# anthonyhu/tumblr-emotions

Hardware: AMD Instinct MI355X
Metric: training samples/sec (224x224 img + 32-tok text, batch 256) (higher is better)
Workload: dtype f32; 1 GPU; joint train step (fwd+bwd+all-reduce+Adam): Inception-v1 224x224x3 + 300-d embedding + LSTM-512, T=32, V=10000, 15 classes, batch 256 per GPU, reference freeze (<=Mixed_5b conv weights frozen, all BN betas trainable), dropout 0.8, BN train mode; global_batch=256, per_gpu_batch=256, parallelism=dp1, launch=eager

## Files before the change

### include/ds_kernels.h

```cpp
#ifndef DS_KERNELS_H
#define DS_KERNELS_H

#include <stddef.h>
#include <stdint.h>

#ifdef __cplusplus
extern "C" {
#endif

#define DS_OK 0
#define DS_ERR_ARG (-1)
#define DS_ERR_LAUNCH (-2)
#define DS_ERR_WORKSPACE (-3)

#define DS_DTYPE_F32 0
#define DS_DTYPE_BF16 1

#define DS_EPI_BIAS 1
#define DS_EPI_RELU 2
#define DS_EPI_ACCUM 4
#define DS_EPI_STATS 8
#define DS_EPI_MASK 16
#define DS_EPI_BNSUMS 32
#define DS_EPI_BN_RELU 64
// ... 20 lines not shown
    int32_t splits;
    int64_t z_split_stride;
    int32_t tile_nt;
    int32_t grid_x;
    int32_t dtype;
    int32_t x_dtype;
    int32_t partials;
    const float *norm_rstd;
    const float *norm_shift;
    const float *mask_rstd;
    const float *mask_shift;
    const struct ds_bn_bwd_on_load *bnb;
    int32_t mask_dtype;
    int32_t z_dtype;
    uint8_t *pool_argmax;
    const struct ds_bn_finalize_in_launch *fin;
} ds_conv_desc;

typedef struct ds_bn_finalize_in_launch {
    const float *beta;
    float *mean, *rstd, *shift;
    float *moving_mean, *moving_var;
    uint32_t *ticket;
    int64_t count;
    float eps, decay;
} ds_bn_finalize_in_launch;

typedef struct ds_bn_bwd_on_load {
    const float *mean, *rstd, *shift;
    const float *coef;
// ... 7 lines not shown
int ds_debug_conv_set_tile(int mt, int nt);
int ds_debug_conv_set_path(int path);
int ds_debug_conv_set_wide(int mode);
int ds_debug_conv_wino_allow_ablation(int on);
int ds_debug_conv_wino4_set_nb(int nb);
int ds_debug_conv_bf16_set_max_nb(int nb);
int ds_debug_conv_wgrad_force(int ai, int bj, int slabs);
int ds_debug_conv_wgrad_plan(const ds_conv_desc *d, const float *x, const float *dz, int32_t lddz, const float *dw,
                             const void *ws, int out[6]);
#endif
int ds_conv_igemm_partials(const ds_conv_desc *d);
int ds_conv_igemm_bnsums_supported(const ds_conv_desc *d);
int ds_conv_igemm_norm_supported(const ds_conv_desc *d);
int ds_conv_igemm_bnb_supported(const ds_conv_desc *d);
int ds_conv_igemm_pool3_supported(const ds_conv_desc *d);
int ds_conv_igemm_finalize_tickets(const ds_conv_desc *d);
int ds_conv_igemm(const ds_conv_desc *d, const float *x, const float *w, float *z, const float *bias,
                  const float *mask, float *stats, const float *pivot, void *stream);

size_t ds_weights_bf16_bytes(int32_t Cin, int32_t Cout, int32_t taps, int32_t dgrad);
int ds_weights_to_bf16(const float *w, void *wb, int32_t Cin, int32_t Cout, int32_t taps, int32_t dgrad, void *stream);
int ds_conv_bf16_supported(const ds_conv_desc *d);
int ds_conv_bf16_partials(const ds_conv_desc *d);
int ds_conv_bf16(const ds_conv_desc *d, const void *x, const void *wb, float *z, const void *mask, float *stats,
                 const float *pivot, void *stream);

size_t ds_weights_f32x3_bytes(int32_t Cin, int32_t Cout, int32_t taps, int32_t dgrad);
int ds_weights_to_f32x3(const float *w, void *wb, int32_t Cin, int32_t Cout, int32_t taps, int32_t dgrad, void *stream);
int ds_conv_f32x3_supported(const ds_conv_desc *d);
int ds_conv_f32x3_partials(const ds_conv_desc *d);
// ... 105 lines not shown
    const float *x_amax;
    const float *wscale;
    const ds_bn_finalize_in_launch *fin;
    void *ws;
    size_t ws_bytes;
    const float *scale;
    const float *shift;
} ds_conv_io;
int ds_conv_plan(ds_conv_layer_plan *plan, int32_t role, int32_t arith, uint32_t options, int32_t N, int32_t H, int32_t W,
                 int32_t w_cin, int32_t w_cout, int32_t k, int32_t stride, int32_t ldx, int32_t ldz, int32_t flags);
int ds_conv_plan_set_flags(ds_conv_layer_plan *plan, int32_t flags);
int ds_conv_plan_enable_bnsums(ds_conv_layer_plan *plan, int32_t ldy);
int ds_conv_plan_norm_supported(const ds_conv_layer_plan *plan);
int ds_conv_plan_bnb_supported(const ds_conv_layer_plan *plan);
int ds_conv_plan_enable_pool3(ds_conv_layer_plan *plan, uint8_t *argmax);
int ds_conv_plan_enable_bn_relu(ds_conv_layer_plan *plan);
int ds_conv_plan_finalize_tickets(const ds_conv_layer_plan *plan);
int ds_conv_prepare_weights(const ds_conv_layer_plan *plan, const float *w_hwio, void *w_prepared, float *wscale,
                            void *stream);
int ds_conv_run(const ds_conv_layer_plan *plan, const void *x, const void *w, float *z, const ds_conv_io *io, void *stream);

size_t ds_conv_wgrad_workspace(const ds_conv_desc *d);
int ds_conv_wgrad(const ds_conv_desc *d, const float *x, const float *dz, int32_t lddz, float *dw,
                  void *ws, size_t ws_bytes, void *stream);

int ds_bn_finalize(const float *stats, int32_t P, int64_t count, int32_t C, const float *beta, const float *pivot,
                   float eps, float decay, float *mean, float *rstd, float *shift, float *moving_mean,
                   float *moving_var, void *stream);

int ds_bn_finalize_centered(const float *stats, int32_t P, int64_t count, int32_t C, const float *beta, const float *pivot,
// ... 349 lines not shown
```

### tumblr_emotions_amd/_lib.py

```python
import ctypes as C
import os

_HERE = os.path.dirname(os.path.abspath(__file__))
LIB_PATH = os.environ.get("DS_LIB") or os.path.join(_HERE, "libds_kernels.so")

def tuning_env(name, default=None):
    return os.environ.get(name, default) if os.environ.get("DS_LIB") else default


DS_EPI_BIAS, DS_EPI_RELU, DS_EPI_ACCUM, DS_EPI_STATS, DS_EPI_MASK, DS_EPI_BNSUMS = 1, 2, 4, 8, 16, 32
DS_EPI_BN_RELU = 64
DS_DTYPE_F32, DS_DTYPE_BF16 = 0, 1
DS_FP8_E4M3, DS_FP8_E5M2 = 0, 1
DS_CONV_FWD, DS_CONV_DGRAD = 0, 1
DS_LSTM_SKIP_MASKED = 256
DS_ARITH_F32, DS_ARITH_BF16, DS_ARITH_FP8, DS_ARITH_F32X3 = 0, 1, 2, 3
DS_FAM_IGEMM, DS_FAM_WINO2, DS_FAM_WINO4, DS_FAM_STEM, DS_FAM_BF16D, DS_FAM_FP8D, DS_FAM_F32X3, DS_FAM_WINO4H, DS_FAM_STEM_POOL = range(9)
DS_FAM_STEM_DGRAD = 9
DS_PLAN_NO_WINO, DS_PLAN_NO_WINO4, DS_PLAN_NO_STEM_DIRECT, DS_PLAN_NO_BF16_DIRECT, DS_PLAN_ACT16, DS_PLAN_PACKED_RGB = 1, 2, 4, 8, 16, 32
DS_PLAN_FP8_EVERYWHERE, DS_PLAN_FP8_WIDE_RULE, DS_PLAN_NO_WINO4H, DS_PLAN_STEM_POOL = 64, 128, 256, 512
DS_PLAN_NO_SPLITK = 1024
DS_PREPROCESS_FLIP, DS_PREPROCESS_SATURATION_FIRST = 1, 2
DS_JPEG_UNSUPPORTED, DS_JPEG_MORE = 1, 2
DS_JPEG_444, DS_JPEG_422, DS_JPEG_420, DS_JPEG_GREY = 0, 1, 2, 3
DS_JPEG_E_CODE, DS_JPEG_E_RUN, DS_JPEG_E_RANGE, DS_JPEG_E_COLUMN, DS_JPEG_E_SEGMENT, DS_JPEG_E_TABLE = 1, 2, 4, 8, 16, 32


class ConvDesc(C.Structure):
    _fields_ = [
        ("N", C.c_int32), ("H", C.c_int32), ("W", C.c_int32), ("Cin", C.c_int32), ("ldx", C.c_int32),
        ("KH", C.c_int32), ("KW", C.c_int32), ("stride", C.c_int32), ("pad_t", C.c_int32), ("pad_l", C.c_int32),
        ("OH", C.c_int32), ("OW", C.c_int32), ("Cout", C.c_int32), ("ldz", C.c_int32),
        ("w_tap_stride", C.c_int64), ("w_n_stride", C.c_int32), ("w_k_stride", C.c_int32),
        ("flip", C.c_int32), ("fold_cin", C.c_int32), ("flags", C.c_int32), ("ldmask", C.c_int32),
        ("splits", C.c_int32), ("z_split_stride", C.c_int64),
        ("tile_nt", C.c_int32), ("grid_x", C.c_int32), ("dtype", C.c_int32), ("x_dtype", C.c_int32),
        ("partials", C.c_int32),
        ("norm_rstd", C.c_void_p), ("norm_shift", C.c_void_p), ("mask_rstd", C.c_void_p), ("mask_shift", C.c_void_p),
        ("bnb", C.c_void_p), ("mask_dtype", C.c_int32), ("z_dtype", C.c_int32), ("pool_argmax", C.c_void_p), ("fin", C.c_void_p),
    ]


class BnBwdOnLoad(C.Structure):
    _fields_ = [("mean", C.c_void_p), ("rstd", C.c_void_p), ("shift", C.c_void_p), ("coef", C.c_void_p),
                ("nseg", C.c_int32), ("c_end", C.c_int32 * 3), ("ld", C.c_int32 * 3), ("dy", C.c_void_p * 3)]


class BnFinalizeInLaunch(C.Structure):
    _fields_ = [("beta", C.c_void_p), ("mean", C.c_void_p), ("rstd", C.c_void_p), ("shift", C.c_void_p),
                ("moving_mean", C.c_void_p), ("moving_var", C.c_void_p), ("ticket", C.c_void_p), ("count", C.c_int64),
                ("eps", C.c_float), ("decay", C.c_float)]


class LayerPlanStruct(C.Structure):
# ... 90 lines not shown
_i32, _i64, _f32, _u64 = C.c_int32, C.c_int64, C.c_float, C.c_uint64
_CD = C.POINTER(ConvDesc)
_SG = C.POINTER(Segments)
_SS = C.POINTER(SumSegments)
_LP = C.POINTER(LayerPlanStruct)
_IO = C.POINTER(ConvIO)

SIGNATURES = {
    "ds_version": (C.c_int, []),
    "ds_last_error": (C.c_char_p, []),
    "ds_conv_igemm_partials": (C.c_int, [_CD]),
    "ds_conv_igemm_bnsums_supported": (C.c_int, [_CD]),
    "ds_conv_igemm_norm_supported": (C.c_int, [_CD]),
    "ds_conv_igemm_bnb_supported": (C.c_int, [_CD]),
    "ds_conv_igemm_pool3_supported": (C.c_int, [_CD]),
    "ds_conv_igemm_finalize_tickets": (C.c_int, [_CD]),
    "ds_conv_igemm": (C.c_int, [_CD, _P, _P, _P, _P, _P, _P, _P, _P]),
    "ds_weights_bf16_bytes": (C.c_size_t, [_i32, _i32, _i32, _i32]),
    "ds_weights_to_bf16": (C.c_int, [_P, _P, _i32, _i32, _i32, _i32, _P]),
    "ds_conv_bf16_supported": (C.c_int, [_CD]),
    "ds_conv_bf16_partials": (C.c_int, [_CD]),
    "ds_conv_bf16": (C.c_int, [_CD, _P, _P, _P, _P, _P, _P, _P]),
    "ds_weights_f32x3_bytes": (C.c_size_t, [_i32, _i32, _i32, _i32]),
    "ds_weights_to_f32x3": (C.c_int, [_P, _P, _i32, _i32, _i32, _i32, _P]),
    "ds_conv_f32x3_supported": (C.c_int, [_CD]),
    "ds_conv_f32x3_partials": (C.c_int, [_CD]),
    "ds_conv_f32x3": (C.c_int, [_CD, _P, _P, _P, _P, _P, _P, _P]),
    "ds_absmax": (C.c_int, [_P, _i64, _i32, _P, _P]),
    "ds_weights_fp8_bytes": (C.c_size_t, [_i32, _i32, _i32, _i32]),
    "ds_weights_to_fp8": (C.c_int, [_P, _P, _P, _i32, _i32, _i32, _i32, _P]),
# ... 19 lines not shown
    "ds_conv_wino4_partials": (C.c_int, [_i32, _i32, _i32]),
    "ds_conv_wino4_splitk_choose": (C.c_int, [_i32, _i32, _i32, _i32, _i32]),
    "ds_conv_wino4_splitk_partials": (C.c_int, [_i32, _i32, _i32]),
    "ds_conv_wino4_splitk_workspace": (C.c_size_t, [_i32, _i32, _i32, _i32, _i32]),
    "ds_conv_wino4_splitk": (C.c_int, [_P, _P, _P, _P, _P, _P, _i32, _i32, _i32, _i32, _i32, _i32, _i32, _i32, _i32, _i32, _P, C.c_size_t, _P]),
    "ds_conv_wino4": (C.c_int, [_P, _P, _P, _P, _P, _P, _i32, _i32, _i32, _i32, _i32, _i32, _i32, _i32, _P]),
    "ds_conv_wino4_bf16x2": (C.c_int, [_P, _P, _P, _P, _P, _P, _i32, _i32, _i32, _i32, _i32, _i32, _i32, _i32, _i32, _P]),
    "ds_conv_wino4_bf16x2_x16": (C.c_int, [_P, _P, _P, _P, _P, _P, _i32, _i32, _i32, _i32, _i32, _i32, _i32, _i32, _i32, _P]),
    "ds_wino4_transform_weights_bf16x2": (C.c_int, [_P, _P, _i32, _i32, _i32, _P]),
    "ds_conv_plan": (C.c_int, [_LP, _i32, _i32, C.c_uint32] + [_i32] * 10),
    "ds_conv_plan_set_flags": (C.c_int, [_LP, _i32]),
    "ds_conv_plan_enable_bnsums": (C.c_int, [_LP, _i32]),
    "ds_conv_plan_norm_supported": (C.c_int, [_LP]),
    "ds_conv_plan_bnb_supported": (C.c_int, [_LP]),
    "ds_conv_plan_enable_pool3": (C.c_int, [_LP, C.c_void_p]),
    "ds_conv_plan_enable_bn_relu": (C.c_int, [_LP]),
    "ds_conv_plan_finalize_tickets": (C.c_int, [_LP]),
    "ds_conv_prepare_weights": (C.c_int, [_LP, _P, _P, _P, _P]),
    "ds_conv_run": (C.c_int, [_LP, _P, _P, _P, _IO, _P]),
    "ds_conv_wgrad_workspace": (C.c_size_t, [_CD]),
    "ds_conv_wgrad": (C.c_int, [_CD, _P, _P, _i32, _P, _P, C.c_size_t, _P]),
    "ds_bn_finalize": (C.c_int, [_P, _i32, _i64, _i32, _P, _P, _f32, _f32, _P, _P, _P, _P, _P, _P]),
    "ds_bn_finalize_centered": (C.c_int, [_P, _i32, _i64, _i32, _P, _P, _f32, _f32, _P, _P, _P, _P, _P, _P, _P, _P]),
    "ds_bn_apply_relu": (C.c_int, [_P, _i64, _i32, _P, _P, _SG, _P]),
    "ds_bn_apply_relu_z16": (C.c_int, [_P, _i64, _i32, _P, _P, _SG, _P]),
    "ds_bn_bwd_apply_z16": (C.c_int, [_P, _i32, _SG, _i64, _i32, _P, _P, _P, _P, _P, _i32, _P, _P]),
    "ds_bn_infer_prepare": (C.c_int, [_P, _P, _P, _f32, _i32, _P, _P, _P]),
    "ds_bn_infer_prepare_multi": (C.c_int, [_P, _i32, _f32, _P]),
    "ds_bn_bwd_partials": (C.c_int, [_i64, _i32]),
    "ds_bn_bwd_reduce": (C.c_int, [_P, _i32, _i32, _SG, _i64, _i32, _P, _P, _P, _P, _P]),
# ... 152 lines not shown
```

### tumblr_emotions_amd/csrc/conv_igemm.hip

```cpp
#include <stdlib.h>
#include <mutex>
#include <type_traits>
#include <unordered_map>
#include "conv_epilogue.h"

using ds::f32x16;
typedef float f32x4 __attribute__((ext_vector_type(4)));
typedef float f32x2 __attribute__((ext_vector_type(2)));
typedef unsigned int u32x4 __attribute__((ext_vector_type(4)));
typedef __attribute__((address_space(3))) void *lds_ptr;

namespace {

constexpr int BK = 16;
constexpr int LDK = 20;
using ds::kOOB;
using ds::make_srd;

struct ConvParams {
    ds_conv_desc d;
    const float *x;
    const float *w;
    float *z;
    const float *bias;
    const float *mask;
// ... 1813 lines not shown
    if (d->splits <= 1) p.d.z_split_stride = 0;
    p.x = (const float *)x; p.w = (const float *)w; p.z = z; p.mask = (const float *)mask; p.stats = stats;
    p.pivot = (d->flags & DS_EPI_STATS) ? pivot : nullptr;
    p.M = (int)conv_M(d);
    p.taps = d->KH * d->KW;
    const int64_t x_elems = ((int64_t)d->N * d->H * d->W - 1) * d->ldx + (d->fold_cin > 0 ? d->fold_cin : d->Cin);
    const int64_t w_elems = (int64_t)(p.taps - 1) * d->w_tap_stride + (int64_t)(d->Cout - 1) * d->w_n_stride +
                            (int64_t)(d->Cin - 1) * d->w_k_stride + 1;
    const int64_t w_bytes = prepared_w_bytes < 0 ? w_elems * 4 : prepared_w_bytes;
    DS_REQUIRE(x_elems * 4 < (1ll << 31) && w_bytes < (1ll << 31), "%s: operand larger than 2 GiB%s", who, hint);
    p.x_bytes = (unsigned)(x_elems * 4);
    p.w_bytes = (unsigned)w_bytes;
    return DS_OK;
}

int igemm_launch(const ds_conv_desc *d, const float *x, const float *w, float *z, const float *bias, const float *mask,
                 float *stats, const float *pivot, const float *scale, const float *shift, void *stream) {
    DS_REQUIRE(d && x && w && z, "ds_conv_igemm: null argument");
    DS_REQUIRE(d->Cin > 0 && d->Cout > 0 && d->N > 0 && d->OH > 0 && d->OW > 0, "ds_conv_igemm: bad dims");
    DS_REQUIRE(d->w_n_stride == 1 || d->w_k_stride == 1, "ds_conv_igemm: one weight stride must be 1");
    DS_REQUIRE(!(d->flags & DS_EPI_BIAS) || bias, "ds_conv_igemm: DS_EPI_BIAS without bias");
    DS_REQUIRE(!(d->flags & DS_EPI_MASK) || mask, "ds_conv_igemm: DS_EPI_MASK without mask");
    DS_REQUIRE(!(d->flags & DS_EPI_STATS) || stats, "ds_conv_igemm: DS_EPI_STATS without stats buffer");
    DS_REQUIRE(!(d->flags & DS_EPI_BNSUMS) || (stats && mask && !(d->flags & (DS_EPI_STATS | DS_EPI_MASK)) && d->ldmask >= d->Cout),
               "ds_conv_igemm: DS_EPI_BNSUMS needs the partials buffer (stats), y (mask, ldmask) and excludes STATS / MASK");
    DS_REQUIRE(conv_M(d) < (1ll << 31), "ds_conv_igemm: M too large");
    DS_REQUIRE(d->dtype == DS_DTYPE_F32 || d->dtype == DS_DTYPE_BF16, "ds_conv_igemm: dtype must be DS_DTYPE_F32 or DS_DTYPE_BF16");
    const Launch L = choose(d, aligned16(x, w));
    const Variant &v = L.v;
    const TileCfg &c = L.c;
    DS_REQUIRE(!(d->flags & DS_EPI_STATS) || v.vec == dims_vec(d),
               "ds_conv_igemm: DS_EPI_STATS needs 16-byte aligned operand pointers");

    ConvParams p;
// ... 89 lines not shown
extern "C" int ds_conv_igemm_bnsums_supported(const ds_conv_desc *d) {
    if (!d) return 0;
    ds_conv_desc t = *d;
    t.flags = (t.flags & DS_EPI_ACCUM) | DS_EPI_BNSUMS;
    return choose(&t, true).c.wide > 0 ? 1 : 0;
}

extern "C" int ds_conv_igemm_norm_supported(const ds_conv_desc *d) {
    if (!d || d->Cin > 1024) return 0;
    return choose(d, true).c.wide > 0 ? 1 : 0;
}

extern "C" int ds_conv_igemm_pool3_supported(const ds_conv_desc *d) {
    if (!d) return 0;
    return choose(d, true, kBeforePool).c.wide > 0 ? 1 : 0;
}

extern "C" int ds_conv_igemm_finalize_tickets(const ds_conv_desc *d) {
    if (!d || !(d->flags & DS_EPI_STATS)) return 0;
    ds_conv_desc t = *d;
    t.partials = 0;
    t.fin = nullptr;
    const Launch L = choose(&t, true);
    return L.c.wide && L.row_tiles <= 256 ? L.gy : 0;
}

namespace ds {
int conv_igemm_bn_relu_supported(const ds_conv_desc *d) {
    if (!d || (d->flags & ~DS_EPI_BN_RELU)) return 0;
    ds_conv_desc t = *d;
// ... 184 lines not shown
```

### tumblr_emotions_amd/csrc/conv_plan.cpp

```cpp
#include <stdlib.h>
#include <string.h>

#include "ds_kernels.h"

namespace ds {
void set_error(const char *fmt, ...);
int conv_igemm_bn_relu_supported(const ds_conv_desc *d);
int conv_igemm_bn_relu(const ds_conv_desc *d, const float *x, const float *w, float *z, const float *scale, const float *shift,
                       void *stream);
int conv_wino_bn_relu(const float *x, const float *u, float *z, const float *scale, const float *shift, int32_t N, int32_t H,
                      int32_t W, int32_t Cin, int32_t ldx, int32_t Cout, int32_t ldz, void *stream);
int conv_wino4_bn_relu(const float *x, const float *u, float *z, const float *scale, const float *shift, int32_t N, int32_t H,
                       int32_t W, int32_t Cin, int32_t ldx, int32_t Cout, int32_t ldz, int32_t splits, void *ws, size_t ws_bytes,
                       void *stream);
}

#define PLAN_REQUIRE(cond, ...)         \
    do {                                \
        if (!(cond)) {                  \
            ds::set_error(__VA_ARGS__); \
            return DS_ERR_ARG;          \
        }                               \
    } while (0)

namespace {

// ... 205 lines not shown
extern "C" int ds_conv_plan_bnb_supported(const ds_conv_layer_plan *p) {
    if (p == nullptr || p->role != DS_CONV_DGRAD || p->family != DS_FAM_IGEMM || p->k != 1) return 0;
    const ds_conv_desc t = igemm_desc(p);
    return ds_conv_igemm_bnb_supported(&t);
}

extern "C" int ds_conv_plan_enable_pool3(ds_conv_layer_plan *p, uint8_t *argmax) {
    if (p == nullptr || argmax == nullptr || p->role != DS_CONV_FWD || p->family != DS_FAM_IGEMM || p->k != 1) return 0;
    const ds_conv_desc t = igemm_desc(p);
    if (!ds_conv_igemm_pool3_supported(&t)) return 0;
    p->d.pool_argmax = argmax;
    recount_partials(p);
    return 1;
}

extern "C" int ds_conv_plan_enable_bn_relu(ds_conv_layer_plan *p) {
    if (p == nullptr || p->role != DS_CONV_FWD || p->d.dtype != DS_DTYPE_F32 || p->d.flags != 0) return 0;
    if (p->family == DS_FAM_IGEMM) {
        const ds_conv_desc t = igemm_desc(p);
        if (!ds::conv_igemm_bn_relu_supported(&t)) return 0;
    } else if (p->family == DS_FAM_WINO4) {
        if (p->d.ldz % 4 != 0 || p->d.ldz < p->d.Cout) return 0;
    } else if (p->family != DS_FAM_WINO2) {
        return 0;
    }
    p->d.flags = DS_EPI_BN_RELU;
    p->d.partials = 0;
    p->partials = 0;
    return 1;
}
// ... 98 lines not shown
```

### tumblr_emotions_amd/engine_image.py

```python
import contextlib
import ctypes as C
import os
from collections import namedtuple

import torch

from . import _lib, ops
from .ops import WgradPlan, gemm_plan, make_segments, same_pad, DS_EPI_BIAS, DS_EPI_STATS

BN_EPS = 0.001
BN_DECAY = 0.9997
WEIGHT_DECAY = 0.00004

TOPOLOGY = [
    ("conv", "Conv2d_1a_7x7", 7, 2, 64),
    ("maxpool", "MaxPool_2a_3x3", 3, 2),
    ("conv", "Conv2d_2b_1x1", 1, 1, 64),
    ("conv", "Conv2d_2c_3x3", 3, 1, 192),
    ("maxpool", "MaxPool_3a_3x3", 3, 2),
    ("mixed", "Mixed_3b", 64, (96, 128), (16, 32), 32),
    ("mixed", "Mixed_3c", 128, (128, 192), (32, 96), 64),
    ("maxpool", "MaxPool_4a_3x3", 3, 2),
    ("mixed", "Mixed_4b", 192, (96, 208), (16, 48), 64),
    ("mixed", "Mixed_4c", 160, (112, 224), (24, 64), 64),
# ... 745 lines not shown
        b0, b1a, b1b, b2a, b2b, b3 = self.b
        cin, Ct = self.prev.C, self.C
        self.B = B
        M = B * self.H * self.W
        for l in self.layers:
            l.alloc(B)
        out16 = eng.act16 and self.name not in ("Mixed_5b", "Mixed_5c")
        r16 = eng.act16 and self.name != "Mixed_5c"
        a16 = lambda f: torch.bfloat16 if f else torch.float32
        self.out = torch.empty(B, self.H, self.W, Ct, device=dev, dtype=a16(out16))
        self.dout = torch.empty(B, self.H, self.W, Ct, device=dev)
        self.r1 = torch.empty(M, b1a, device=dev, dtype=a16(r16))
        self.r2 = torch.empty(M, b2a, device=dev, dtype=a16(r16))
        self.dr1 = torch.empty(M, b1a, device=dev)
        self.dr2 = torch.empty(M, b2a, device=dev)
        self.dpooled = torch.empty(M, cin, device=dev)
        self.argmax = torch.empty(M, cin, dtype=torch.uint8, device=dev)
        self.fuse_b3 = bool(eng.fuse_branch3 and not self.c3.trainable and eng.dtype == "f32" and not eng.act16
                            and self.c3.fwd.enable_pool3(self.argmax))
        if self.fuse_b3:
            eng.need_stats(self.c3.fwd.partials * 2 * b3)
        self.pooled = None if self.fuse_b3 else torch.empty(M, cin, device=dev, dtype=self.prev.out.dtype)
        o, do = self.out.data_ptr(), self.dout.data_ptr()
        nf = b0 + b1a + b2a
        es, dt_o, dt_r = self.out.element_size(), ops.act_dtype(self.out), ops.act_dtype(self.r1)
        self.out_amax, self.r1_amax, self.r2_amax = eng.new_amax(), eng.new_amax(), eng.new_amax()
        am_o, am_1, am_2 = ops._p(self.out_amax), ops._p(self.r1_amax), ops._p(self.r2_amax)
        self.seg_f = make_segments([(0, b0, o, Ct, dt_o, am_o), (b0, b0 + b1a, self.r1.data_ptr(), b1a, dt_r, am_1),
                                    (b0 + b1a, nf, self.r2.data_ptr(), b2a, dt_r, am_2)])
        self.seg_1, self.seg_2, self.seg_3 = (make_segments([(0, layer.cout, o + es * off, Ct, dt_o, am_o)])
                                              for layer, off in self.concat_layers()[1:])
# ... 30 lines not shown
        self.fused.make_dgrad(cin, allow_z16=True)
        self.c1.make_dgrad(b1a, allow_z16=True)
        self.c2.make_dgrad(b2a, allow_z16=True)
        self.c3.make_dgrad(cin, allow_z16=True)
        self.dpooled16 = bool(eng.dpooled16 and eng.act16 and self.c3.dgrad.family == ops.DS_FAM_BF16D)
        if self.dpooled16:
            self.dpooled = torch.empty(M, cin, device=dev, dtype=torch.bfloat16)
            self.c3.dgrad.d.z_dtype = ops.DS_DTYPE_BF16
        for part, (layer, r) in enumerate(((self.c1, self.r1), (self.c2, self.r2)), start=1):
            src = layer.emit_dx_sums(r)
            if src is not None:
                self.fused.sums_from(part, src)
        p = self.prev
        fams = (ops.DS_FAM_IGEMM, ops.DS_FAM_BF16D, ops.DS_FAM_FP8D) if _lib.tuning_env("DS_POOL_FIRST_16") == "1" else (ops.DS_FAM_IGEMM,)
        self.pool_first = bool(eng.pool_first and self.fused.dgrad.family in fams)
        if isinstance(p, MixedStage) and self.pool_first:
            src = self.fused.emit_dx_sums(p.out)
            if src is not None and p.zcat:
                self.fused.dgrad.d.mask_rstd = p.rs_cat[0].data_ptr()
                self.fused.dgrad.d.mask_shift = p.rs_cat[1].data_ptr()
            if src is not None:
                for layer, off in p.concat_layers():
                    layer.sums_from(0, src._replace(off=off))
        self.pool_sums = None
        self.split_dout = False
        if isinstance(p, MixedStage) and not self.pool_first and eng.bwd_sums and eng.pool_sums and cin <= 1024 \
                and not p.zcat:
            P = ops.maxpool3_bwd_sums_partials(B, p.W, cin)
            self.pool_sums = torch.empty(2 * cin * P, device=dev)
            src, delta = None, 0
# ... 122 lines not shown
        if self.eng.fuse_fin_apply:
            ops.bn_bwd_finalize_apply(sg, M, Cb, None, None, self.coef_cat, z, dy, self.mean_cat[b0:], self.rs_cat[0, b0:],
                                      self.rs_cat[1, b0:], z, self.fa_ticket, ldz=Ct, betas=[l.beta for l in layers],
                                      dbetas=[l.gbeta for l in layers])
        else:
            ops.bn_bwd_finalize_multi(sg, M, Cb, [l.beta for l in layers], [l.gbeta for l in layers], self.coef_cat)
            if from_pool:
                nx = self.next
                ops.bn_pool_bwd_apply_cols(z, Ct, z, Ct, nx.dout, nx.argmax, Ct, b0, self.B, self.H, self.W, Cb, self.mean_cat[b0:],
                                           self.rs_cat[0, b0:], self.rs_cat[1, b0:], self.coef_cat[0], self.coef_cat[1], nx.k)
            else:
                ops.bn_bwd_apply(z, dy, M, Cb, self.mean_cat[b0:], self.rs_cat[0, b0:], self.rs_cat[1, b0:], self.coef_cat, z, ldz=Ct)
        for l in layers:
            l._dz_amax_live = False

    def forward(self):
        p = self.prev
        b0, b1a, b1b, b2a, b2b, b3 = self.b
        x = ops._p(p.out)
        dx_, dr_ = ops.act_dtype(p.out), ops.act_dtype(self.r1)
        ax_, a1_, a2_ = p.out_amax, self.r1_amax, self.r2_amax
        defer = self._batch_forward()

        def branch3():
            self._pool_fwd()
            self.c3.forward(x if self.fuse_b3 else ops._p(self.pooled), p.C, self.seg_3, dx_, ax_, defer)

        self._fork_join(lambda: self.fused.forward(x, p.C, self.seg_f, dx_, ax_),
                        lambda: self.c1.forward(ops._p(self.r1), b1a, self.seg_1, dr_, a1_, defer),
                        lambda: self.c2.forward(ops._p(self.r2), b2a, self.seg_2, dr_, a2_, defer), branch3)
# ... 31 lines not shown
                        l.fz_job = (self._fz_close.data_ptr() + 4 * off * P, P)
                        off += l.cout
                ops.bn_infer_bwd_apply_sums(z, dy, M, Ct - b0, self.rs_cat[0, b0:], self.rs_cat[1, b0:], z, self._fz_close, ldz=Ct)
            else:
                ops.bn_infer_bwd_apply(z, dy, M, Ct - b0, self.rs_cat[0, b0:], self.rs_cat[1, b0:], z, ldz=Ct)

        def closing(layer, x_ptr, ldx, dx_ptr, ndx):
            if infer:
                layer.backward_pointwise(x_ptr, ldx, dx_ptr, ndx, apply=not self.zcat)
            elif batched:
                layer._run_dgrad(dx_ptr)
            else:
                layer.backward(x_ptr, ldx, dx_ptr, ndx)

        def branch3():
            closing(self.c3, None if self.fuse_b3 else ops._p(self.pooled), p.C, ops._p(self.dpooled), need_dx)
            if pool_first:
                ops.maxpool_bwd(self.dpooled, self.argmax, p.dout, False, self.B, p.H, p.W, p.C, 3, 1, "SAME")
            elif need_dx and self.split_dout and infer:
                ops.maxpool_bwd(self.dpooled, self.argmax, p.dout2, False, self.B, p.H, p.W, p.C, 3, 1, "SAME")
            elif need_dx and self.split_dout:
                ops.maxpool3_bwd_sums(self.dpooled, self.argmax, p.dout2, False, p.out, self.B, p.H, p.W, p.C, self.pool_sums)

        self._fork_join(None, lambda: closing(self.c1, ops._p(self.r1), b1a, ops._p(self.dr1), True),
                        lambda: closing(self.c2, ops._p(self.r2), b2a, ops._p(self.dr2), True), branch3)
        if infer:
            self.fused.backward_pointwise(x, p.C, ops._p(p.dout) if need_dx else None, need_dx)
            if need_dx and not pool_first and not self.split_dout:
                ops.maxpool_bwd(self.dpooled, self.argmax, p.dout, True, self.B, p.H, p.W, p.C, 3, 1, "SAME")
            return
        self.fused.backward(x, p.C, ops._p(p.dout) if need_dx else None, need_dx, pool=self.next if from_pool else None)
        if need_dx and self.split_dout:
            ops.bn_bwd_reduce(p.out, self._dgrad_sum_segs, self.B * p.H * p.W, p.C, eng.zeros, eng.ones, eng.zeros, self.dgrad_sums,
                              ldz=p.C)
        if need_dx and not pool_first and not self.split_dout:
            if self.pool_sums is not None:
                ops.maxpool3_bwd_sums(self.dpooled, self.argmax, p.dout, True, p.out, self.B, p.H, p.W, p.C, self.pool_sums)
            else:
                ops.maxpool_bwd(self.dpooled, self.argmax, p.dout, True, self.B, p.H, p.W, p.C, 3, 1, "SAME")


class InceptionV1Engine:

    def __init__(self, store, num_classes, image_size=224, dropout_keep_prob=0.8, trainable_bn_beta=True,
                 device="cuda", train_all=False, dtype="f32"):
        self.store, self.num_classes, self.keep = store, num_classes, dropout_keep_prob
        assert dtype in ("f32", "bf16", "fp8")
        self.dtype = dtype
        self.conv_dtype = ops.DS_DTYPE_F32 if dtype == "f32" else ops.DS_DTYPE_BF16
        self.trainable_bn_beta = trainable_bn_beta
        self.train_all = train_all
        self.device = torch.device(device)
        self.update_moving = True
        self.training = True
# ... 22 lines not shown
        self.winograd = True
        self.mul3 = _lib.tuning_env("DS_MUL3", "0") == "1"
        self.bnb_on_load = int(_lib.tuning_env("DS_BNB", "1"))
        self.zcat = _lib.tuning_env("DS_ZCAT", "1") != "0"
        self.pool_apply = _lib.tuning_env("DS_POOL_APPLY", "1") != "0"
        self.fuse_finalize = _lib.tuning_env("DS_FUSE_FIN", "0") == "1"
        self.fuse_fin_apply = _lib.tuning_env("DS_FIN_APPLY", "0") == "1"
        e = _lib.tuning_env("DS_BATCH_BN")
        self.batch_bn = int(e) if e else None
        self.pool_sums = _lib.tuning_env("DS_POOL_SUMS", "1") != "0"
        self.split_dout = _lib.tuning_env("DS_SPLIT_DOUT", "0") == "1"
        self.z16 = _lib.tuning_env("DS_Z16", "1") != "0"
        self.dpooled16 = _lib.tuning_env("DS_DPOOLED16", "0") == "1"
        self.stem_sums_from_dgrad = _lib.tuning_env("DS_STEM_SUMS", "1") != "0"
        self.dz16 = int(_lib.tuning_env("DS_DZ16", "2"))
        self.fuse_branch3 = _lib.tuning_env("DS_FUSE_B3", "1") != "0"
        self.winograd4 = _lib.tuning_env("DS_WINO4", "1") != "0"
        self.splitk = _lib.tuning_env("DS_SPLITK", "1") != "0"
        e = _lib.tuning_env("DS_TEXT_GATE")
        self.text_gate = int(e) if e else None
        self.text_gate_event = None
        self.weights_version = 0
        self.fused_infer = False
        self._fused_key = None
        self._fused_targets = {}
        self._fused_jobs = None
        self.input_grad = False
        self.infer_bwd = False
        self.frozen_step = False
        self._frozen_prep = None
# ... 448 lines not shown
```

### tumblr_emotions_amd/ops.py

```python
import ctypes as C
import os

import torch

from . import _lib
from ._lib import (ConvDesc, Segments, SumSegments, DS_EPI_ACCUM, DS_EPI_BIAS, DS_EPI_BNSUMS, DS_EPI_MASK, DS_EPI_RELU,
                   DS_EPI_STATS, DS_EPI_BN_RELU,
                   DS_DTYPE_BF16, DS_DTYPE_F32, DS_FP8_E4M3, DS_FP8_E5M2, DS_CONV_FWD, DS_CONV_DGRAD, DS_ARITH_F32, DS_ARITH_BF16,
                   DS_ARITH_FP8, DS_ARITH_F32X3, DS_FAM_IGEMM, DS_FAM_WINO2, DS_FAM_WINO4, DS_FAM_STEM, DS_FAM_BF16D, DS_FAM_FP8D,
                   DS_FAM_F32X3, DS_FAM_WINO4H, DS_FAM_STEM_POOL, DS_FAM_STEM_DGRAD, DS_PLAN_STEM_POOL, DS_PLAN_NO_SPLITK, DS_PLAN_NO_WINO4H, DS_PLAN_NO_WINO, DS_PLAN_NO_WINO4, DS_PLAN_NO_STEM_DIRECT, DS_PLAN_NO_BF16_DIRECT, DS_PLAN_ACT16,
                   DS_PLAN_PACKED_RGB, DS_PLAN_FP8_EVERYWHERE, DS_PLAN_FP8_WIDE_RULE)


_raw_stream = getattr(torch._C, "_cuda_getCurrentRawStream", None)


def _stream():
    if _raw_stream is not None:
        return C.c_void_p(_raw_stream(torch.cuda.current_device()))
    return C.c_void_p(torch.cuda.current_stream().cuda_stream)


def _p(t):
    if t is None:
# ... 73 lines not shown

class ConvTimer:

    def __init__(self):
        self.records = []
        self._start = None

    def begin(self):
        self._start = torch.cuda.Event(enable_timing=True)
        self._start.record(torch.cuda.current_stream())

    def end(self, plan):
        e = torch.cuda.Event(enable_timing=True)
        e.record(torch.cuda.current_stream())
        d = getattr(plan, "d", None)
        pooled = getattr(plan, "family", None) == DS_FAM_STEM_POOL or bool(getattr(d, "pool_argmax", None))
        self.records.append((self._start, e, plan.alg_flops, pooled))

    def summary(self, pooled=None):
        recs = [r for r in self.records if pooled is None or r[3] == pooled]
        ms = sum(s.elapsed_time(e) for (s, e, _, _) in recs)
        return len(recs), ms, sum(f for (_, _, f, _) in recs)


CONV_TIMER = None


def head_gemm_plan(M, K, N, lda, ldc, w_ld, transposed_w=False, flags=0, ldmask=0, *, device):
    if M <= 512 and K >= 256 and _lib.tuning_env("DS_SPLIT_GEMM", "1") != "0":
        return SplitGemm(M, K, N, lda, ldc, w_ld, transposed_w, flags, ldmask, 8 if K >= 512 else 4, device)
    return gemm_plan(M, K, N, lda, ldc, w_ld, transposed_w=transposed_w, flags=flags, ldmask=ldmask)
# ... 168 lines not shown
            _lib.check(_lib.load().ds_conv_prepare_weights(self._ref, w_hwio, _p(self.u), _p(self.wscale), _stream()),
                       "ds_conv_prepare_weights")

    def enable_bnsums(self, ldy):
        return int(_lib.load().ds_conv_plan_enable_bnsums(self._ref, ldy))

    def norm_supported(self):
        return bool(_lib.load().ds_conv_plan_norm_supported(self._ref))

    def enable_pool3(self, argmax):
        if not _lib.load().ds_conv_plan_enable_pool3(self._ref, _p(argmax)):
            return False
        self.pool_argmax = argmax
        return True

    def copy(self):
        q = object.__new__(LayerPlan)
        q.p = _lib.LayerPlanStruct()
        C.memmove(C.byref(q.p), self._ref, C.sizeof(q.p))
        q._ref = C.byref(q.p)
        q.d, q.family, q.M, q.alg_flops = q.p.d, q.p.family, self.M, self.alg_flops
        q.u, q.wscale, q._ws = self.u, self.wscale, self._ws
        q.io = _lib.ConvIO()
        q.io.ws, q.io.ws_bytes = self.io.ws, self.io.ws_bytes
        q.ws_bytes, q.splitk = self.ws_bytes, self.splitk
        q._run, q._io_ref = self._run, C.byref(q.io)
        q.pool_argmax = getattr(self, "pool_argmax", None)
        return q

    def bn_relu_variant(self, ldz=None):
        q = self.copy()
        q.p.d.flags, q.p.d.partials, q.p.partials = 0, 0, 0
        if ldz is not None:
            q.p.d.ldz = ldz
        if not _lib.load().ds_conv_plan_enable_bn_relu(q._ref):
            return None
        return q

    def run_bn_relu(self, x, w_hwio, y, scale, shift):
        t = CONV_TIMER
        if t is not None:
            t.begin()
# ... 1182 lines not shown
```

Baseline: 20410 samples/s.

## Fuse 1x1 branch-3 dgrad with 3x3 maxpool backward in Inception blocks

Adds a new HIP kernel that computes the branch-3 1x1 conv input gradient with MFMA and immediately scatters it through the stored 3x3 maxpool argmax into the previous stage's dout. This skips writing and re-reading the intermediate dpooled buffer and drops the separate maxpool_bwd launch. The plan enables it only for small-channel fp32 IGEMM dgrad layers with enough tasks. The cost is a more complex kernel with a rolling row-window scheme whose occupancy and correctness depend on map width of at most 32.

```diff
diff --git a/include/ds_kernels.h b/include/ds_kernels.h
--- a/include/ds_kernels.h
+++ b/include/ds_kernels.h
@@ -58,6 +58,7 @@
     int32_t mask_dtype;
     int32_t z_dtype;
     uint8_t *pool_argmax;
+    const uint8_t *pool_bwd_argmax;
     const struct ds_bn_finalize_in_launch *fin;
 } ds_conv_desc;
 
@@ -95,6 +96,7 @@
 int ds_conv_igemm_norm_supported(const ds_conv_desc *d);
 int ds_conv_igemm_bnb_supported(const ds_conv_desc *d);
 int ds_conv_igemm_pool3_supported(const ds_conv_desc *d);
+int ds_conv_igemm_pool3_bwd_supported(const ds_conv_desc *d);
 int ds_conv_igemm_finalize_tickets(const ds_conv_desc *d);
 int ds_conv_igemm(const ds_conv_desc *d, const float *x, const float *w, float *z, const float *bias,
                   const float *mask, float *stats, const float *pivot, void *stream);
@@ -230,6 +232,7 @@
 int ds_conv_plan_norm_supported(const ds_conv_layer_plan *plan);
 int ds_conv_plan_bnb_supported(const ds_conv_layer_plan *plan);
 int ds_conv_plan_enable_pool3(ds_conv_layer_plan *plan, uint8_t *argmax);
+int ds_conv_plan_enable_pool3_bwd(ds_conv_layer_plan *plan, const uint8_t *argmax);
 int ds_conv_plan_enable_bn_relu(ds_conv_layer_plan *plan);
 int ds_conv_plan_finalize_tickets(const ds_conv_layer_plan *plan);
 int ds_conv_prepare_weights(const ds_conv_layer_plan *plan, const float *w_hwio, void *w_prepared, float *wscale,
diff --git a/tumblr_emotions_amd/_lib.py b/tumblr_emotions_amd/_lib.py
--- a/tumblr_emotions_amd/_lib.py
+++ b/tumblr_emotions_amd/_lib.py
@@ -37,7 +37,8 @@
         ("tile_nt", C.c_int32), ("grid_x", C.c_int32), ("dtype", C.c_int32), ("x_dtype", C.c_int32),
         ("partials", C.c_int32),
         ("norm_rstd", C.c_void_p), ("norm_shift", C.c_void_p), ("mask_rstd", C.c_void_p), ("mask_shift", C.c_void_p),
-        ("bnb", C.c_void_p), ("mask_dtype", C.c_int32), ("z_dtype", C.c_int32), ("pool_argmax", C.c_void_p), ("fin", C.c_void_p),
+        ("bnb", C.c_void_p), ("mask_dtype", C.c_int32), ("z_dtype", C.c_int32), ("pool_argmax", C.c_void_p),
+        ("pool_bwd_argmax", C.c_void_p), ("fin", C.c_void_p),
     ]
 
 
@@ -158,6 +159,7 @@
     "ds_conv_igemm_norm_supported": (C.c_int, [_CD]),
     "ds_conv_igemm_bnb_supported": (C.c_int, [_CD]),
     "ds_conv_igemm_pool3_supported": (C.c_int, [_CD]),
+    "ds_conv_igemm_pool3_bwd_supported": (C.c_int, [_CD]),
     "ds_conv_igemm_finalize_tickets": (C.c_int, [_CD]),
     "ds_conv_igemm": (C.c_int, [_CD, _P, _P, _P, _P, _P, _P, _P, _P]),
     "ds_weights_bf16_bytes": (C.c_size_t, [_i32, _i32, _i32, _i32]),
@@ -207,6 +209,7 @@
     "ds_conv_plan_norm_supported": (C.c_int, [_LP]),
     "ds_conv_plan_bnb_supported": (C.c_int, [_LP]),
     "ds_conv_plan_enable_pool3": (C.c_int, [_LP, C.c_void_p]),
+    "ds_conv_plan_enable_pool3_bwd": (C.c_int, [_LP, C.c_void_p]),
     "ds_conv_plan_enable_bn_relu": (C.c_int, [_LP]),
     "ds_conv_plan_finalize_tickets": (C.c_int, [_LP]),
     "ds_conv_prepare_weights": (C.c_int, [_LP, _P, _P, _P, _P]),
diff --git a/tumblr_emotions_amd/csrc/conv_igemm.hip b/tumblr_emotions_amd/csrc/conv_igemm.hip
--- a/tumblr_emotions_amd/csrc/conv_igemm.hip
+++ b/tumblr_emotions_amd/csrc/conv_igemm.hip
@@ -9,6 +9,11 @@
 typedef float f32x2 __attribute__((ext_vector_type(2)));
 typedef unsigned int u32x4 __attribute__((ext_vector_type(4)));
 typedef __attribute__((address_space(3))) void *lds_ptr;
+
+namespace ds {
+int conv_pool3_bwd_shape_ok(const ds_conv_desc *d);
+int conv_pool3_bwd(const ds_conv_desc *d, const float *dz, const float *w, float *dx, int tile_order, void *stream);
+}
 
 namespace {
 
@@ -1852,10 +1857,25 @@
     return DS_OK;
 }
 
+int pool3_bwd_form(const ds_conv_desc *d, bool aligned) {
+    if (!ds::conv_pool3_bwd_shape_ok(d)) return 0;
+    ds_conv_desc t = *d;
+    t.pool_bwd_argmax = nullptr;
+    const Launch L = choose(&t, aligned);
+    if (L.c.wide) return 1;
+    return (L.c.direct || L.c.glds || L.c.bf16 || L.v.fold) ? 0 : 2;
+}
+
 int igemm_launch(const ds_conv_desc *d, const float *x, const float *w, float *z, const float *bias, const float *mask,
                  float *stats, const float *pivot, const float *scale, const float *shift, void *stream) {
     DS_REQUIRE(d && x && w && z, "ds_conv_igemm: null argument");
     DS_REQUIRE(d->Cin > 0 && d->Cout > 0 && d->N > 0 && d->OH > 0 && d->OW > 0, "ds_conv_igemm: bad dims");
+    if (d->pool_bwd_argmax) {
+        const int form = pool3_bwd_form(d, aligned16(x, w));
+        DS_REQUIRE(form > 0, "ds_conv_igemm: ds_conv_desc.pool_bwd_argmax on a descriptor the launch is not built for "
+                             "(ds_conv_igemm_pool3_bwd_supported)");
+        return ds::conv_pool3_bwd(d, x, w, z, form == 2, stream);
+    }
     DS_REQUIRE(d->w_n_stride == 1 || d->w_k_stride == 1, "ds_conv_igemm: one weight stride must be 1");
     DS_REQUIRE(!(d->flags & DS_EPI_BIAS) || bias, "ds_conv_igemm: DS_EPI_BIAS without bias");
     DS_REQUIRE(!(d->flags & DS_EPI_MASK) || mask, "ds_conv_igemm: DS_EPI_MASK without mask");
@@ -1975,6 +1995,10 @@
 extern "C" int ds_conv_igemm_pool3_supported(const ds_conv_desc *d) {
     if (!d) return 0;
     return choose(d, true, kBeforePool).c.wide > 0 ? 1 : 0;
+}
+
+extern "C" int ds_conv_igemm_pool3_bwd_supported(const ds_conv_desc *d) {
+    return pool3_bwd_form(d, true) > 0 ? 1 : 0;
 }
 
 extern "C" int ds_conv_igemm_finalize_tickets(const ds_conv_desc *d) {
diff --git a/tumblr_emotions_amd/csrc/conv_plan.cpp b/tumblr_emotions_amd/csrc/conv_plan.cpp
--- a/tumblr_emotions_amd/csrc/conv_plan.cpp
+++ b/tumblr_emotions_amd/csrc/conv_plan.cpp
@@ -10,6 +10,7 @@
                        void *stream);
 int conv_wino_bn_relu(const float *x, const float *u, float *z, const float *scale, const float *shift, int32_t N, int32_t H,
                       int32_t W, int32_t Cin, int32_t ldx, int32_t Cout, int32_t ldz, void *stream);
+int64_t conv_pool3_bwd_tasks(const ds_conv_desc *d, int *rpb, int *grp_rows, int *gpi, int *ncb);
 int conv_wino4_bn_relu(const float *x, const float *u, float *z, const float *scale, const float *shift, int32_t N, int32_t H,
                        int32_t W, int32_t Cin, int32_t ldx, int32_t Cout, int32_t ldz, int32_t splits, void *ws, size_t ws_bytes,
                        void *stream);
@@ -245,6 +246,17 @@
     return 1;
 }
 
+extern "C" int ds_conv_plan_enable_pool3_bwd(ds_conv_layer_plan *p, const uint8_t *argmax) {
+    if (p == nullptr || argmax == nullptr || p->role != DS_CONV_DGRAD || p->family != DS_FAM_IGEMM || p->k != 1) return 0;
+    const ds_conv_desc t = igemm_desc(p);
+    if (!ds_conv_igemm_pool3_bwd_supported(&t)) return 0;
+    if (p->d.Cin > 64) return 0;
+    int rpb, grp_rows, gpi, ncb;
+    if (ds::conv_pool3_bwd_tasks(&t, &rpb, &grp_rows, &gpi, &ncb) < 1024) return 0;
+    p->d.pool_bwd_argmax = argmax;
+    return 1;
+}
+
 extern "C" int ds_conv_plan_enable_bn_relu(ds_conv_layer_plan *p) {
     if (p == nullptr || p->role != DS_CONV_FWD || p->d.dtype != DS_DTYPE_F32 || p->d.flags != 0) return 0;
     if (p->family == DS_FAM_IGEMM) {
diff --git a/tumblr_emotions_amd/csrc/conv_pool_bwd.hip b/tumblr_emotions_amd/csrc/conv_pool_bwd.hip
--- /dev/null
+++ b/tumblr_emotions_amd/csrc/conv_pool_bwd.hip
@@ -0,0 +1,204 @@
+#include "conv_epilogue.h"
+
+typedef float f32x4 __attribute__((ext_vector_type(4)));
+typedef unsigned int u32x4 __attribute__((ext_vector_type(4)));
+using ds::f32x16;
+using ds::kOOB;
+using ds::make_srd;
+
+namespace {
+
+struct PoolBwdParams {
+    const float *dz;
+    const float *w;
+    const uint8_t *am;
+    float *dx;
+    int N, H, W, K, C;
+    int lddz, ldw, lddx;
+    int rpb;
+    int grp_rows, gpi;
+    int ncb, tasks;
+    int tile_order;
+    unsigned dz_bytes, w_bytes, am_bytes, dx_bytes;
+};
+
+constexpr int TP = 36;
+constexpr int WAVE_LDS = 32 * TP + 32 * 8;
+
+template <int KS>
+__global__ __launch_bounds__(256, KS <= 1 ? 4 : (KS <= 4 ? 3 : 2)) void pool3_bwd_dgrad_kernel(const PoolBwdParams p) {
+    __shared__ __attribute__((aligned(16))) float smem[4 * WAVE_LDS];
+    const int lane = threadIdx.x & 63;
+    const int wave = __builtin_amdgcn_readfirstlane((int)threadIdx.x >> 6);
+    const int task = (int)blockIdx.x * 4 + wave;
+    if (task >= p.tasks) return;
+    const int g = task / p.ncb, cb = task - g * p.ncb;
+    const int n = g / p.gpi, gi = g - n * p.gpi;
+    const int W = p.W, H = p.H;
+    const int h0 = gi * p.grp_rows, h1 = min(H, h0 + p.grp_rows);
+    const int c_lo = max(h0 - 1, 0), c_hi = min(h1 + 1, H);
+    const int n0 = cb * 32;
+    const int li = lane & 31, kh = lane >> 5;
+    float *tile = smem + wave * WAVE_LDS;
+    unsigned *amt = reinterpret_cast<unsigned *>(tile + 32 * TP);
+    const __amdgpu_buffer_rsrc_t srd_dz = make_srd(p.dz, p.dz_bytes), srd_w = make_srd(p.w, p.w_bytes);
+    const __amdgpu_buffer_rsrc_t srd_am = make_srd(p.am, p.am_bytes), srd_dx = make_srd(p.dx, p.dx_bytes);
+
+    const unsigned k0 = p.tile_order ? 8u * kh : 4u * kh;
+    const int k1 = p.tile_order ? 16 : 32;
+    const unsigned wo = n0 + li < p.C ? ((unsigned)(n0 + li) * (unsigned)p.ldw + k0) * 4u : kOOB;
+    f32x4 blo[KS], bhi[KS];
+#pragma unroll
+    for (int ks = 0; ks < KS; ++ks) {
+        blo[ks] = __builtin_bit_cast(f32x4, __builtin_amdgcn_raw_buffer_load_b128(srd_w, wo, ks * 64, 0));
+        bhi[ks] = __builtin_bit_cast(f32x4, __builtin_amdgcn_raw_buffer_load_b128(srd_w, wo, ks * 64 + k1, 0));
+    }
+
+    f32x4 a0[KS], a1[KS];
+    u32x4 wn;
+    auto request = [&](int crow0) {
+        const int cnt = min(p.rpb, c_hi - crow0) * W;
+        const int mbase = (n * H + crow0) * W;
+        const unsigned vo = li < cnt ? ((unsigned)(mbase + li) * (unsigned)p.lddz + k0) * 4u : kOOB;
+#pragma unroll
+        for (int ks = 0; ks < KS; ++ks) {
+            a0[ks] = __builtin_bit_cast(f32x4, __builtin_amdgcn_raw_buffer_load_b128(srd_dz, vo, ks * 64, 0));
+            a1[ks] = __builtin_bit_cast(f32x4, __builtin_amdgcn_raw_buffer_load_b128(srd_dz, vo, ks * 64 + k1, 0));
+        }
+        const int px = lane >> 1, hf = lane & 1;
+        const unsigned va = (px < cnt && n0 + 16 * hf < p.C) ? (unsigned)(mbase + px) * (unsigned)p.C + (unsigned)(n0 + 16 * hf) : kOOB;
+        wn = __builtin_bit_cast(u32x4, __builtin_amdgcn_raw_buffer_load_b128(srd_am, va, 0, 0));
+    };
+
+    const int q = lane & 7, wl = lane >> 3;
+    const bool colok = n0 + 4 * q < p.C;
+    f32x4 accP[4], accC[4];
+#pragma unroll
+    for (int ps = 0; ps < 4; ++ps) accP[ps] = accC[ps] = f32x4{0.f, 0.f, 0.f, 0.f};
+    auto store_row = [&](int hs, int w, const f32x4 &v) {
+        const unsigned vz = ((unsigned)((n * H + hs) * W + w) * (unsigned)p.lddx + (unsigned)(n0 + 4 * q)) * 4u;
+        __builtin_amdgcn_raw_buffer_store_b128(__builtin_bit_cast(u32x4, v), srd_dx, vz, 0, 0);
+    };
+
+    request(c_lo);
+    for (int crow0 = c_lo; crow0 < c_hi; crow0 += p.rpb) {
+        const int nrows = min(p.rpb, c_hi - crow0);
+        f32x16 acc;
+#pragma unroll
+        for (int e = 0; e < 16; ++e) acc[e] = 0.f;
+#pragma unroll
+        for (int ks = 0; ks < KS; ++ks) {
+#pragma unroll
+            for (int j = 0; j < 4; ++j) acc = __builtin_amdgcn_mfma_f32_32x32x2f32(a0[ks][j], blo[ks][j], acc, 0, 0, 0);
+#pragma unroll
+            for (int j = 0; j < 4; ++j) acc = __builtin_amdgcn_mfma_f32_32x32x2f32(a1[ks][j], bhi[ks][j], acc, 0, 0, 0);
+        }
+        const u32x4 wcur = wn;
+        if (crow0 + p.rpb < c_hi) request(crow0 + p.rpb);
+        asm volatile("s_waitcnt lgkmcnt(0)" ::: "memory");
+#pragma unroll
+        for (int e = 0; e < 16; ++e) tile[(ds::acc_row(e) + 4 * kh) * TP + li] = acc[e];
+        *reinterpret_cast<u32x4 *>(amt + (lane >> 1) * 8 + (lane & 1) * 4) = wcur;
+        asm volatile("s_waitcnt lgkmcnt(0)" ::: "memory");
+        for (int r = 0; r < nrows; ++r) {
+            const int oh = crow0 + r;
+            const bool st = oh - 1 >= h0 && oh - 1 < h1;
+#pragma unroll
+            for (int ps = 0; ps < 4; ++ps) {
+                if (ps * 8 < W) {
+                    const int w = ps * 8 + wl;
+                    const bool act = w < W;
+                    f32x4 sN = {0.f, 0.f, 0.f, 0.f}, sC = accC[ps], sP = accP[ps];
+#pragma unroll
+                    for (int qq = 0; qq < 3; ++qq) {
+                        const int ow = w - 1 + qq;
+                        const bool ok = act && ow >= 0 && ow < W;
+                        const int slot = ok ? r * W + ow : 0;
+                        const f32x4 dv = *reinterpret_cast<const f32x4 *>(tile + slot * TP + 4 * q);
+                        const unsigned a = ok ? amt[slot * 8 + q] : 0xFFFFFFFFu;
+#pragma unroll
+                        for (int j = 0; j < 4; ++j) {
+                            const unsigned b = (a >> (8 * j)) & 0xFFu;
+                            sN[j] += b == (unsigned)(6 + 2 - qq) ? dv[j] : 0.f;
+                            sC[j] += b == (unsigned)(3 + 2 - qq) ? dv[j] : 0.f;
+                            sP[j] += b == (unsigned)(2 - qq) ? dv[j] : 0.f;
+                        }
+                    }
+                    if (st && act && colok) store_row(oh - 1, w, sP);
+                    accP[ps] = sC;
+                    accC[ps] = sN;
+                }
+            }
+        }
+    }
+    if (c_hi == h1) {
+#pragma unroll
+        for (int ps = 0; ps < 4; ++ps) {
+            const int w = ps * 8 + wl;
+            if (w < W && colok) store_row(h1 - 1, w, accP[ps]);
+        }
+    }
+}
+
+typedef void (*PoolBwdFn)(const PoolBwdParams);
+
+PoolBwdFn kernel_for(int K) {
+    switch (K) {
+    case 16: return pool3_bwd_dgrad_kernel<1>;
+    case 32: return pool3_bwd_dgrad_kernel<2>;
+    case 64: return pool3_bwd_dgrad_kernel<4>;
+    case 128: return pool3_bwd_dgrad_kernel<8>;
+    default: return nullptr;
+    }
+}
+
+}
+
+namespace ds {
+
+int conv_pool3_bwd_shape_ok(const ds_conv_desc *d) {
+    if (!d || d->dtype != DS_DTYPE_F32 || d->x_dtype != DS_DTYPE_F32 || d->z_dtype != DS_DTYPE_F32) return 0;
+    if (d->KH != 1 || d->KW != 1 || d->stride != 1 || d->fold_cin || d->splits > 1 || d->OH != d->H || d->OW != d->W) return 0;
+    if (d->flags != 0 || d->bnb || d->fin || d->norm_rstd || d->norm_shift || d->pool_argmax) return 0;
+    if (d->w_k_stride != 1 || d->w_n_stride < d->Cin || d->w_n_stride % 4 != 0) return 0;
+    if (d->N < 1 || d->H < 1 || d->W < 1 || d->W > 32 || d->Cout < 16 || d->Cout % 16 != 0 || !kernel_for(d->Cin)) return 0;
+    if (d->ldx % 4 != 0 || d->ldx < d->Cin || d->ldz % 4 != 0 || d->ldz < d->Cout) return 0;
+    const int64_t M = (int64_t)d->N * d->H * d->W;
+    if (((M - 1) * d->ldx + d->Cin) * 4 >= (1ll << 31) || ((M - 1) * d->ldz + d->Cout) * 4 >= (1ll << 31) || M * d->Cout >= (1ll << 31))
+        return 0;
+    return 1;
+}
+
+int64_t conv_pool3_bwd_tasks(const ds_conv_desc *d, int *rpb, int *grp_rows, int *gpi, int *ncb) {
+    *rpb = 32 / d->W;
+    *grp_rows = (d->H + *rpb - 1) / *rpb <= 8 ? d->H : 14 * *rpb;
+    *gpi = (d->H + *grp_rows - 1) / *grp_rows;
+    *ncb = (d->Cout + 31) / 32;
+    return (int64_t)d->N * *gpi * *ncb;
+}
+
+int conv_pool3_bwd(const ds_conv_desc *d, const float *dz, const float *w, float *dx, int tile_order, void *stream) {
+    DS_REQUIRE(d && dz && w && dx && d->pool_bwd_argmax, "ds_conv_igemm: pool_bwd_argmax launch with a null argument");
+    DS_REQUIRE(conv_pool3_bwd_shape_ok(d),
+               "ds_conv_igemm: ds_conv_desc.pool_bwd_argmax is implemented for the fp32 1x1 stride-1 Conv2DBackpropInput on maps at most "
+               "32 wide, Cout %% 16 == 0, Cin in {16, 32, 64, 128}, without epilogue flags (ds_conv_igemm_pool3_bwd_supported)");
+    DS_REQUIRE(((((uintptr_t)dz | (uintptr_t)w | (uintptr_t)dx | (uintptr_t)d->pool_bwd_argmax)) & 15) == 0,
+               "ds_conv_igemm: pool_bwd_argmax needs 16-byte aligned operands");
+    PoolBwdParams p = {};
+    p.dz = dz; p.w = w; p.am = d->pool_bwd_argmax; p.dx = dx;
+    p.N = d->N; p.H = d->H; p.W = d->W; p.K = d->Cin; p.C = d->Cout;
+    p.lddz = d->ldx; p.ldw = d->w_n_stride; p.lddx = d->ldz;
+    p.tile_order = tile_order;
+    const int64_t tasks = conv_pool3_bwd_tasks(d, &p.rpb, &p.grp_rows, &p.gpi, &p.ncb);
+    DS_REQUIRE(tasks < (1ll << 31), "ds_conv_igemm: pool_bwd_argmax launch too large");
+    p.tasks = (int)tasks;
+    const int64_t M = (int64_t)d->N * d->H * d->W;
+    p.dz_bytes = (unsigned)(((M - 1) * d->ldx + d->Cin) * 4);
+    p.w_bytes = (unsigned)(((int64_t)(d->Cout - 1) * d->w_n_stride + d->Cin) * 4);
+    p.am_bytes = (unsigned)(M * d->Cout);
+    p.dx_bytes = (unsigned)(((M - 1) * d->ldz + d->Cout) * 4);
+    hipLaunchKernelGGL(kernel_for(d->Cin), dim3((unsigned)((tasks + 3) / 4)), dim3(256), 0, (hipStream_t)stream, p);
+    return ds::check_launch("ds_conv_igemm (pool_bwd_argmax)");
+}
+
+}
diff --git a/tumblr_emotions_amd/engine_image.py b/tumblr_emotions_amd/engine_image.py
--- a/tumblr_emotions_amd/engine_image.py
+++ b/tumblr_emotions_amd/engine_image.py
@@ -783,7 +783,7 @@
         self.r2 = torch.empty(M, b2a, device=dev, dtype=a16(r16))
         self.dr1 = torch.empty(M, b1a, device=dev)
         self.dr2 = torch.empty(M, b2a, device=dev)
-        self.dpooled = torch.empty(M, cin, device=dev)
+        self.dpooled = None
         self.argmax = torch.empty(M, cin, dtype=torch.uint8, device=dev)
         self.fuse_b3 = bool(eng.fuse_branch3 and not self.c3.trainable and eng.dtype == "f32" and not eng.act16
                             and self.c3.fwd.enable_pool3(self.argmax))
@@ -844,6 +844,13 @@
         p = self.prev
         fams = (ops.DS_FAM_IGEMM, ops.DS_FAM_BF16D, ops.DS_FAM_FP8D) if _lib.tuning_env("DS_POOL_FIRST_16") == "1" else (ops.DS_FAM_IGEMM,)
         self.pool_first = bool(eng.pool_first and self.fused.dgrad.family in fams)
+        self.fuse_b3_bwd = bool(eng.fuse_b3_bwd and self.pool_first and eng.dtype == "f32" and not eng.act16 and not self.dpooled16
+                                and self.c3.dgrad.family == ops.DS_FAM_IGEMM
+                                and self.c3.dgrad.enable_pool3_bwd(self.argmax, force=eng.fuse_b3_bwd == 2))
+        self._b3_winners = self.argmax.data_ptr()
+        self.c3.dgrad.d.pool_bwd_argmax = None
+        if not self.fuse_b3_bwd and not self.dpooled16:
+            self.dpooled = torch.empty(M, cin, device=dev)
         if isinstance(p, MixedStage) and self.pool_first:
             src = self.fused.emit_dx_sums(p.out)
             if src is not None and p.zcat:
@@ -996,6 +1003,11 @@
         for l in layers:
             l._dz_amax_live = False
 
+    def _dpooled_buf(self):
+        if self.dpooled is None:
+            self.dpooled = torch.empty(self.B * self.H * self.W, self.prev.C, device=self.eng.device)
+        return self.dpooled
+
     def forward(self):
         p = self.prev
         b0, b1a, b1b, b2a, b2b, b3 = self.b
@@ -1057,20 +1069,28 @@
                 layer.backward(x_ptr, ldx, dx_ptr, ndx)
 
         def branch3():
-            closing(self.c3, None if self.fuse_b3 else ops._p(self.pooled), p.C, ops._p(self.dpooled), need_dx)
+            one = pool_first and self.fuse_b3_bwd and not infer
+            dst = p.dout if one else (self._dpooled_buf() if need_dx else self.dpooled)
+            self.c3.dgrad.d.pool_bwd_argmax = self._b3_winners if one else None
+            try:
+                closing(self.c3, None if self.fuse_b3 else ops._p(self.pooled), p.C, ops._p(dst), need_dx)
+            finally:
+                self.c3.dgrad.d.pool_bwd_argmax = None
+            if one:
+                return
             if pool_first:
-                ops.maxpool_bwd(self.dpooled, self.argmax, p.dout, False, self.B, p.H, p.W, p.C, 3, 1, "SAME")
+                ops.maxpool_bwd(dst, self.argmax, p.dout, False, self.B, p.H, p.W, p.C, 3, 1, "SAME")
             elif need_dx and self.split_dout and infer:
-                ops.maxpool_bwd(self.dpooled, self.argmax, p.dout2, False, self.B, p.H, p.W, p.C, 3, 1, "SAME")
+                ops.maxpool_bwd(dst, self.argmax, p.dout2, False, self.B, p.H, p.W, p.C, 3, 1, "SAME")
             elif need_dx and self.split_dout:
-                ops.maxpool3_bwd_sums(self.dpooled, self.argmax, p.dout2, False, p.out, self.B, p.H, p.W, p.C, self.pool_sums)
+                ops.maxpool3_bwd_sums(dst, self.argmax, p.dout2, False, p.out, self.B, p.H, p.W, p.C, self.pool_sums)
 
         self._fork_join(None, lambda: closing(self.c1, ops._p(self.r1), b1a, ops._p(self.dr1), True),
                         lambda: closing(self.c2, ops._p(self.r2), b2a, ops._p(self.dr2), True), branch3)
         if infer:
             self.fused.backward_pointwise(x, p.C, ops._p(p.dout) if need_dx else None, need_dx)
             if need_dx and not pool_first and not self.split_dout:
-                ops.maxpool_bwd(self.dpooled, self.argmax, p.dout, True, self.B, p.H, p.W, p.C, 3, 1, "SAME")
+                ops.maxpool_bwd(self._dpooled_buf(), self.argmax, p.dout, True, self.B, p.H, p.W, p.C, 3, 1, "SAME")
             return
         self.fused.backward(x, p.C, ops._p(p.dout) if need_dx else None, need_dx, pool=self.next if from_pool else None)
         if need_dx and self.split_dout:
@@ -1078,9 +1098,9 @@
                               ldz=p.C)
         if need_dx and not pool_first and not self.split_dout:
             if self.pool_sums is not None:
-                ops.maxpool3_bwd_sums(self.dpooled, self.argmax, p.dout, True, p.out, self.B, p.H, p.W, p.C, self.pool_sums)
+                ops.maxpool3_bwd_sums(self._dpooled_buf(), self.argmax, p.dout, True, p.out, self.B, p.H, p.W, p.C, self.pool_sums)
             else:
-                ops.maxpool_bwd(self.dpooled, self.argmax, p.dout, True, self.B, p.H, p.W, p.C, 3, 1, "SAME")
+                ops.maxpool_bwd(self._dpooled_buf(), self.argmax, p.dout, True, self.B, p.H, p.W, p.C, 3, 1, "SAME")
 
 
 class InceptionV1Engine:
@@ -1133,6 +1153,7 @@
         self.dpooled16 = _lib.tuning_env("DS_DPOOLED16", "0") == "1"
         self.stem_sums_from_dgrad = _lib.tuning_env("DS_STEM_SUMS", "1") != "0"
         self.dz16 = int(_lib.tuning_env("DS_DZ16", "2"))
+        self.fuse_b3_bwd = int(_lib.tuning_env("DS_FUSE_B3_BWD", "1"))
         self.fuse_branch3 = _lib.tuning_env("DS_FUSE_B3", "1") != "0"
         self.winograd4 = _lib.tuning_env("DS_WINO4", "1") != "0"
         self.splitk = _lib.tuning_env("DS_SPLITK", "1") != "0"
diff --git a/tumblr_emotions_amd/ops.py b/tumblr_emotions_amd/ops.py
--- a/tumblr_emotions_amd/ops.py
+++ b/tumblr_emotions_amd/ops.py
@@ -111,7 +111,8 @@
         e = torch.cuda.Event(enable_timing=True)
         e.record(torch.cuda.current_stream())
         d = getattr(plan, "d", None)
-        pooled = getattr(plan, "family", None) == DS_FAM_STEM_POOL or bool(getattr(d, "pool_argmax", None))
+        pooled = getattr(plan, "family", None) == DS_FAM_STEM_POOL or bool(getattr(d, "pool_argmax", None)) \
+            or bool(getattr(d, "pool_bwd_argmax", None))
         self.records.append((self._start, e, plan.alg_flops, pooled))
 
     def summary(self, pooled=None):
@@ -310,6 +311,14 @@
         self.pool_argmax = argmax
         return True
 
+    def enable_pool3_bwd(self, argmax, force=False):
+        if not _lib.load().ds_conv_plan_enable_pool3_bwd(self._ref, _p(argmax)):
+            if not (force and _lib.load().ds_conv_igemm_pool3_bwd_supported(C.byref(self.d))):
+                return False
+            self.d.pool_bwd_argmax = argmax.data_ptr()
+        self.pool_bwd_argmax = argmax
+        return True
+
     def copy(self):
         q = object.__new__(LayerPlan)
         q.p = _lib.LayerPlanStruct()
@@ -322,6 +331,7 @@
         q.ws_bytes, q.splitk = self.ws_bytes, self.splitk
         q._run, q._io_ref = self._run, C.byref(q.io)
         q.pool_argmax = getattr(self, "pool_argmax", None)
+        q.pool_bwd_argmax = getattr(self, "pool_bwd_argmax", None)
         return q
 
     def bn_relu_variant(self, ldz=None):
```

Result: no change. 20600 samples/s, median of 6 (+0.9%).
